# gudgud96/music-fader-nets

Hardware: AMD Instinct MI355X
Metric: event-tokens/sec GM-VAE train, seq256 b256 (higher is better)
Workload: dtype f32/bf16x6; 1 GPU; MusicAttrRegGMVAE train step (fwd+losses+bwd+clip+Adam), hidden 512, z 128, K=2, B=256/GPU, T=256, Tr=64 (BASELINE configs[1]; N>1: DP, RCCL grad all-reduce); global_batch=256, seq_len=256, parallelism=dp1

## Files before the change

### include/fadernets.h

```cpp
#ifndef FADERNETS_H
#define FADERNETS_H

#include <stddef.h>
#include <stdint.h>

#ifdef __cplusplus
extern "C" {
#endif

#define FN_OK 0
#define FN_E_NULL (-1)
#define FN_E_SHAPE (-2)
#define FN_E_ALIGN (-3)
#define FN_E_WORKSPACE (-4)
#define FN_E_COUNT (-5)
#define FN_E_UNSUPPORTED (-6)
#define FN_E_COMM (-7)
#define FN_COMM_ERROR_BASE 2000000

#define FN_MAX_SCANS 8

int fn_version(void);
const char* fn_strerror(int code);

#define FN_GEMM_LEAN 0x10000
#define FN_GEMM_BF16X6 0x20000
#define FN_GEMM_X6_PERWAVE 0x40000
#define FN_GEMM_X6_WIDE 0x80000
#define FN_GEMM_X6_PERTILE 0x100000
size_t fn_gemm_ws_bytes(int M, int N, int splitk);
int fn_gemm_f32(int a_kmajor, int b_kmajor, int M, int N, int K, float alpha,
                const float* A, int lda, const float* B, int ldb, float beta, float* C, int ldc,
                const float* bias, int splitk, float* ws, size_t ws_bytes, void* stream);

typedef struct FnGemmSeg {
    const float* A;
    int32_t lda;
    const float* B;
    int32_t ldb;
    int32_t K;
} FnGemmSeg;
typedef struct FnGemmJob {
    int32_t M, N;
    FnGemmSeg seg[4];
    int32_t n_seg;
    float beta;
    float* C;
    int32_t ldc;
// ... 332 lines not shown
```

### music-fader-nets_amd/_lib.py

```python
import ctypes as C
import os

_HERE = os.path.dirname(os.path.abspath(__file__))
LIB_PATH = os.path.join(_HERE, "libfadernets_hip.so")

FN_MAX_SCANS = 8
ABI_VERSION = 6
GEMM_LEAN = 0x10000
GEMM_BF16X6 = 0x20000
GEMM_X6_WIDE = 0x80000
GEMM_X6_PERTILE = 0x100000
GEMM_X6_PERWAVE = 0x40000
GRU_ROWS_MASK = 0xFF
GRU_ALT_TILING = 0x100
GRU_SYNC_ZEROED = 0x200
GRU_COMPILER_LOOPS = 0x400
GRU_NO_PINGPONG = 0x800
GRU_SPREAD_XCDS = 0x1000
GRU_NO_RS_BWD = 0x2000
GRU_BF16X6 = 0x4000
GRU_X6_SINGLE_GROUP = 0x8000
GRU_X6_BWD_32ROWS = 0x8000
FN_E_NULL, FN_E_SHAPE, FN_E_ALIGN, FN_E_WORKSPACE, FN_E_COUNT = -1, -2, -3, -4, -5
FN_E_UNSUPPORTED = -6
# ... 99 lines not shown


class FnNoteParams(C.Structure):
    _fields_ = [("on_lo", C.c_int32), ("off_lo", C.c_int32), ("n_pitch", C.c_int32), ("shift_lo", C.c_int32), ("n_shift", C.c_int32), ("eos", C.c_int32),
                ("vocab_size", C.c_int32), ("vel_lo", C.c_int32), ("n_vel", C.c_int32), ("default_vel", C.c_int32), ("pad", C.c_int32),
                ("add_eos", C.c_int32), ("reserved", C.c_int32 * 4)]


SIGNATURES = {
    "fn_version": (C.c_int, []),
    "fn_strerror": (C.c_char_p, [C.c_int]),
    "fn_frag3_pack": (C.c_int, [vp, C.c_int, C.c_int, C.c_int, vp, vp]),
    "fn_gemm_ws_bytes": (C.c_size_t, [C.c_int, C.c_int, C.c_int]),
    "fn_gemm_f32": (C.c_int, [C.c_int, C.c_int, C.c_int, C.c_int, C.c_int, C.c_float, vp, C.c_int, vp, C.c_int,
                              C.c_float, vp, C.c_int, vp, C.c_int, vp, C.c_size_t, vp]),
    "fn_gemm_multi": (C.c_int, [C.c_int, C.c_int, C.POINTER(FnGemmJob), C.c_int, vp]),
    "fn_transpose_f32": (C.c_int, [vp, C.c_int, C.c_int, C.c_int, vp, C.c_int, vp]),
    "fn_colsum_ws_bytes": (C.c_size_t, [C.c_int, C.c_int]),
    "fn_colsum_f32": (C.c_int, [vp, C.c_int, C.c_int, C.c_int, C.c_float, vp, vp, C.c_size_t, vp]),
    "fn_colsum_multi": (C.c_int, [C.POINTER(FnColsumJob), C.c_int, vp]),
    "fn_axpy_f32": (C.c_int, [C.c_int64, C.c_float, vp, vp, vp]),
    "fn_sum_f32": (C.c_int, [vp, C.c_int64, C.c_float, vp, vp]),
    "fn_gru_gates_floats": (C.c_size_t, [C.c_int, C.c_int]),
    "fn_frag_floats": (C.c_size_t, [C.c_int, C.c_int]),
    "fn_frag_pack": (C.c_int, [vp, C.c_int, C.c_int, C.c_int, vp, vp]),
    "fn_weight_images": (C.c_int, [C.POINTER(FnWeightImage), C.c_int, vp]),
    "fn_gru_sync_ws_bytes": (C.c_size_t, []),
    "fn_gru_seq_fwd": (C.c_int, [C.POINTER(FnGruFwd), C.c_int, vp]),
    "fn_gru_fwd_x6_ok": (C.c_int, [C.POINTER(FnGruFwd), C.c_int]),
    "fn_gru_cell_f32": (C.c_int, [C.POINTER(FnGruCell), vp]),
# ... 85 lines not shown
```

### music-fader-nets_amd/csrc/gemm.hip

```cpp
#include <type_traits>
#include <utility>

#include "common.h"
#include "mma_core.h"
#include "x6w_core.h"

namespace {

constexpr int NT = 256;
constexpr int PF_DEPTH = 2;

template <int BM, int BN, int BK, int WM, int WN, bool AKC, bool BKC>
__global__ __launch_bounds__(NT) void gemm_kernel(int M, int N, int K, float alpha, const float* __restrict__ A, long lda,
                                                  const float* __restrict__ B, long ldb, float beta, float* __restrict__ C,
                                                  long ldc, const float* __restrict__ bias, int ksplit_len,
                                                  float* __restrict__ slabs) {
    constexpr int TM = BM / WM / 16, TN = BN / WN / 16;
    using SA = Stage<BM, BK, AKC, NT>;
    using SB = Stage<BN, BK, BKC, NT>;
    extern __shared__ __attribute__((aligned(16))) float smem[];

    const int ntn = (N + BN - 1) / BN, ntm = (M + BM - 1) / BM;
    const int tile = fn_xcd_remap(blockIdx.x, ntn * ntm);
    const int tm = tile / ntn, tn = tile % ntn;
// ... 525 lines not shown
        for (int e = 0; e < 4; ++e) x6w_cut_row<RN>(dst, e, fa[decltype(SET)::value]);
    };
    auto fused = [&](auto LS, int lblk, auto CS, int, int stage) __attribute__((always_inline)) {
        const float* p0 = base + 32 * lblk;
        u32x4* dst = lds + stage * X6W_STAGE + ps * X6W_SET + r + 16 * q;
#pragma unroll
        for (int e = 0; e < 4; ++e) {
            ld_row(LS, p0, e);
            x6w_cut_row<RN>(dst, e, fa[decltype(CS)::value]);
            __builtin_amdgcn_sched_barrier(0);
        }
    };
    x6w_trips<NS, 2, false>(nblk, request, cut, fused);
}

__global__ __launch_bounds__(X6W_NT) void gemm_nt_x6w_kernel(int M, int N, int K, float alpha, const float* __restrict__ A, long lda,
                                                              const float* __restrict__ B, long ldb, float beta, float* __restrict__ C, long ldc,
                                                              const float* __restrict__ bias) {
    extern __shared__ __attribute__((aligned(16))) u32x4 x6w_lds[];
    const int ntn = N >> 7, ntiles = ntn * (M >> 7);
    const int lane = threadIdx.x & 63, wave = __builtin_amdgcn_readfirstlane(threadIdx.x >> 6);
    const int nblk = K >> 5;
    if (wave >= 4) {
        const int ps = wave & 3;
#pragma unroll 1
        for (int v = blockIdx.x; v < ntiles; v += gridDim.x) {
            const int tile = fn_xcd_remap(v, ntiles);
            const int mb = (tile / ntn) * 128, nb = (tile % ntn) * 128;
            if (ps < 2) x6w_produce_nt<false>(x6w_lds, A + (long)(mb + 64 * ps) * lda, lda, ps, lane, nblk);
            else x6w_produce_nt<true>(x6w_lds, B + (long)(nb + 64 * (ps - 2)) * ldb, ldb, ps, lane, nblk);
        }
        return;
    }
    const int wm = (wave >> 1) & 1, wn = wave & 1;
    const int li = lane & 15, lg = lane >> 4;
#pragma unroll 1
    for (int v = blockIdx.x; v < ntiles; v += gridDim.x) {
        const int tile = fn_xcd_remap(v, ntiles);
        const int mb = (tile / ntn) * 128, nb = (tile % ntn) * 128;
        f32x4 acc[4][4];
#pragma unroll
        for (int a = 0; a < 4; ++a)
#pragma unroll
            for (int b = 0; b < 4; ++b) acc[a][b] = (f32x4){0.f, 0.f, 0.f, 0.f};
// ... 629 lines not shown
                           B, (long)ldb, beta, C, (long)ldc, bias, klen, slabs);                                           \
    }
    if (ak && bk) FN_GEMM_LAUNCH(true, true)
    else if (ak && !bk) FN_GEMM_LAUNCH(true, false)
    else if (!ak && !bk) FN_GEMM_LAUNCH(false, false)
    else FN_GEMM_LAUNCH(false, true)
#undef FN_GEMM_LAUNCH
    FN_CHECK_LAUNCH();
    if (splitk > 1) {
        launch_slab_reduce(st, slabs, splitk, M, N, alpha, beta, C, (long)ldc, bias);
        FN_CHECK_LAUNCH();
    }
    return FN_OK;
}

}

extern "C" {

int fn_out_head_f32(const float* h, int ldh, const float* W, int ldw, const float* bias, int B, int T, int V, int H, const int32_t* target,
                    float grad_scale, float* nll_rows, float* dlogits, int ld, void* stream) {
    if (!h || !W || !bias || !target) return FN_E_NULL;
    if (B <= 0 || T <= 0 || V <= 0 || H <= 0 || ldh < H || ldw < H) return FN_E_SHAPE;
    if (V > OH_BN) return FN_E_UNSUPPORTED;
    if (dlogits && (ld < V || ld > OH_BN || (ld & 3))) return FN_E_SHAPE;
    if (dlogits && (((uintptr_t)dlogits) & 15)) return FN_E_ALIGN;
    const long R = (long)B * T;
    if (R > 0x7fffffff) return FN_E_SHAPE;
    const size_t lds = out_head_lds_bytes();
    if (const int rc = fn_set_max_lds<out_head_kernel>((int)lds, FN_E_SHAPE)) return rc;
// ... 87 lines not shown
        if (rc != FN_OK) return rc;
    } else {
        hipLaunchKernelGGL(f.lean ? gemm_tn_lean_kernel : gemm_tn_kernel, tn_grid(ntm * ntn, splitk), dim3(NT), 0, st, M, N, K, alpha, A, lda, B, ldb, beta, C,
                           ldc, bias, klen, slabs, A2, lda2, msplit);
    }
    FN_CHECK_LAUNCH();
    if (splitk > 1) {
        launch_slab_reduce(st, slabs, splitk, M, N, alpha, beta, C, ldc, bias);
        FN_CHECK_LAUNCH();
    }
    return FN_OK;
}

size_t fn_gemm_ws_bytes(int M, int N, int splitk) { return splitk > 1 ? (size_t)splitk * M * N * sizeof(float) : 0; }

int fn_gemm_f32(int a_kmajor, int b_kmajor, int M, int N, int K, float alpha, const float* A, int lda, const float* B, int ldb,
                float beta, float* C, int ldc, const float* bias, int splitk, float* ws, size_t ws_bytes, void* stream) {
    if (!A || !B || !C) return FN_E_NULL;
    if (M <= 0 || N <= 0 || K <= 0 || lda <= 0 || ldb <= 0 || ldc < N) return FN_E_SHAPE;
    const SplitkFlags f(splitk);
    const bool lean = f.lean, x6 = f.x6;
    const int x6_mode = f.x6_mode;
    splitk = f.splitk;
    if (splitk > 1 && (!ws || ws_bytes < fn_gemm_ws_bytes(M, N, splitk))) return FN_E_WORKSPACE;
    hipStream_t st = (hipStream_t)stream;
    if (!a_kmajor && !b_kmajor && (lda % 4) == 0 && (ldb % 4) == 0 && lda >= 4 && ldb >= 4 &&
        (((((uintptr_t)A) | ((uintptr_t)B)) & 15) == 0))
        return launch_tn(f, st, M, N, K, alpha, A, (long)lda, B, (long)ldb, beta, C, (long)ldc, bias, ws, (const float*)nullptr, 0L, 0);
    if (x6 && a_kmajor && b_kmajor && splitk <= 1 && (M % 128) == 0 && (N % 128) == 0 && (K % 32) == 0 && K >= 128 && (lda % 4) == 0 && (ldb % 4) == 0 &&
        (ldc % 4) == 0 && (((((uintptr_t)A) | ((uintptr_t)B) | ((uintptr_t)C) | ((uintptr_t)bias)) & 15) == 0) && (long)(M / 128) * (N / 128) >= 128) {
        const size_t lds = (size_t)X6W_STAGES * X6W_STAGE * 16;
        if (const int rc = fn_set_max_lds<gemm_nt_x6w_kernel>((int)lds, FN_E_SHAPE)) return rc;
        const int ntiles = (M / 128) * (N / 128), cus = fn_cu_count();
        const int grid = (ntiles > cus && cus >= 8 && (cus & 7) == 0 && !(x6_mode & FN_GEMM_X6_PERTILE)) ? cus : ntiles;
        hipLaunchKernelGGL(gemm_nt_x6w_kernel, dim3(grid), dim3(X6W_NT), lds, st, M, N, K, alpha, A, (long)lda, B, (long)ldb, beta, C, (long)ldc, bias);
        FN_CHECK_LAUNCH();
        return FN_OK;
    }
    if (a_kmajor && b_kmajor && splitk <= 1 && (M % 128) == 0 && (N % 128) == 0 && (K % 16) == 0 && K >= 64 && (lda % 4) == 0 && (ldb % 4) == 0 &&
        (ldc % 4) == 0 && (((((uintptr_t)A) | ((uintptr_t)B) | ((uintptr_t)C) | ((uintptr_t)bias)) & 15) == 0) &&
        (long)M * lda < (1L << 30) && (long)N * ldb < (1L << 30) && (long)(M / 128) * (N / 128) >= 256) {
        if (lean)
            hipLaunchKernelGGL((gemm_nt_direct_kernel<1, 4>), dim3((M / 128) * (N / 128)), dim3(NT), 0, st, M, N, K, alpha, A, (long)lda, B, (long)ldb, beta, C,
                               (long)ldc, bias);
        else
            hipLaunchKernelGGL((gemm_nt_direct_kernel<4, 2>), dim3((M / 128) * (N / 128)), dim3(NT), 0, st, M, N, K, alpha, A, (long)lda, B, (long)ldb, beta, C,
                               (long)ldc, bias);
        FN_CHECK_LAUNCH();
        return FN_OK;
    }
    if (N <= 16 && a_kmajor && b_kmajor && splitk <= 1 && M >= 64)
        return launch_gemm<64, 16, 16, 4, 1>(a_kmajor, b_kmajor, M, N, K, alpha, A, lda, B, ldb, beta, C, ldc, bias, splitk, ws, st);
// ... 91 lines not shown
```

### music-fader-nets_amd/csrc/gru.hip

```cpp
#include <cstdio>

#include "gru_layout.h"
#include "x6w_core.h"

#ifdef FN_TIMING
__device__ unsigned long long fn_dbg[64 * 8];
#define FN_STAMP(k)                                                                                   \
    do {                                                                                              \
        if (blockIdx.x < 64 && threadIdx.x == 0) fn_dbg[blockIdx.x * 8 + (k)] = __builtin_readcyclecounter(); \
    } while (0)
extern "C" int fn_dbg_read(unsigned long long* host) {
    return (int)hipMemcpyFromSymbol(host, HIP_SYMBOL(fn_dbg), sizeof(unsigned long long) * 64 * 8);
}
#else
#define FN_STAMP(k)
#endif

namespace {

constexpr int NT = 256;

struct FwdStep {
    const float* w_frag;
    const float* b_hh;
// ... 378 lines not shown
        for (int e = 0; e < 2; ++e) {
            const float v = x[2 * j + e];
            hi[e] = fn_rn16(v);
            r1[e] = v - hi[e];
            mi[e] = fn_rn16(r1[e]);
            r2[e] = r1[e] - mi[e];
        }
        h[j] = (__float_as_uint(hi[0]) >> 16) | (__float_as_uint(hi[1]) & 0xffff0000u);
        m[j] = (__float_as_uint(mi[0]) >> 16) | (__float_as_uint(mi[1]) & 0xffff0000u);
        l[j] = (__float_as_uint(r2[0]) >> 16) | (__float_as_uint(r2[1]) & 0xffff0000u);
    }
#pragma unroll
    for (int j = 0; j < 4; ++j) { o[j] = h[j]; o[256 + j] = m[j]; o[512 + j] = l[j]; }
}

__global__ void frag3_pack_kernel(const float* __restrict__ src, int rows, int K, long ld, unsigned* __restrict__ dst) {
    const long total = (long)((rows + 15) & ~15) * (K >> 3);
    for (long i = blockIdx.x * (long)blockDim.x + threadIdx.x; i < total; i += (long)gridDim.x * blockDim.x) frag3_item(src, rows, K, ld, 1, dst, i);
}

constexpr int WI_MAX_JOBS = 56;
struct WiJob {
    const float* src;
    float* dst;
    int R, C, ld, kind;
};
struct WiArgs {
    WiJob job[WI_MAX_JOBS];
};

// ... 9 lines not shown
                const int r = r0 + j, c = c0 + tx;
                t[j][tx] = (r < J.R && c < J.C) ? J.src[(long)r * J.ld + c] : 0.f;
            }
            __syncthreads();
            for (int j = ty; j < 32; j += 8) {
                const int c = c0 + j, r = r0 + tx;
                if (r < J.R && c < J.C) J.dst[(long)c * J.R + r] = t[tx][j];
            }
            __syncthreads();
        }
        return;
    }
    if (J.kind == 5) {
        const long total = (long)J.R * J.C;
        for (long i = blockIdx.x * 256L + threadIdx.x; i < total; i += (long)gridDim.x * 256L) J.dst[i] = J.src[(i / J.C) * J.ld + (i % J.C)];
        return;
    }
    if (J.kind >= 3) {
        const int rows = J.kind == 3 ? J.R : J.C, K = J.kind == 3 ? J.C : J.R;
        const long total = (long)((rows + 15) & ~15) * (K >> 3);
        if (J.kind == 3)
            for (long i = blockIdx.x * 256L + threadIdx.x; i < total; i += (long)gridDim.x * 256L)
                frag3_item<false>(J.src, rows, K, (long)J.ld, 1L, reinterpret_cast<unsigned*>(J.dst), i);
        else
            for (long i = blockIdx.x * 256L + threadIdx.x; i < total; i += (long)gridDim.x * 256L)
                frag3_item<true>(J.src, rows, K, 1L, (long)J.ld, reinterpret_cast<unsigned*>(J.dst), i);
        return;
    }
    const int rows = J.kind == 1 ? J.R : J.C, K = J.kind == 1 ? J.C : J.R;
    const int rows16 = (rows + 15) & ~15, NC = K >> 5;
// ... 943 lines not shown
    auto k = gru_cell_kernel<BM, WM, WN>;
    if (const int rc = fn_set_max_lds<gru_cell_kernel<BM, WM, WN>>((int)lds, FN_E_SHAPE)) return rc;
    const int tiles = ((a.B + BM - 1) / BM) * (a.H / 32);
    hipLaunchKernelGGL(k, dim3(tiles), dim3(NT), lds, st, a);
    FN_CHECK_LAUNCH();
    return FN_OK;
}

extern "C" int fn_weight_images(const FnWeightImage* jobs, int n_jobs, void* stream) {
    if (!jobs) return FN_E_NULL;
    if (n_jobs <= 0 || n_jobs > WI_MAX_JOBS) return FN_E_COUNT;
    WiArgs a;
    for (int j = 0; j < n_jobs; ++j) {
        const FnWeightImage& d = jobs[j];
        if (!d.src || !d.dst) return FN_E_NULL;
        if (d.rows <= 0 || d.cols <= 0 || d.ld < d.cols || d.kind < 0 || d.kind > 5) return FN_E_SHAPE;
        if ((d.kind == 1 || d.kind == 3) && (d.cols % 32)) return FN_E_SHAPE;
        if ((d.kind == 2 || d.kind == 4) && (d.rows % 32)) return FN_E_SHAPE;
        if (d.kind != 0 && (((uintptr_t)d.dst) & 15)) return FN_E_ALIGN;
        a.job[j] = WiJob{d.src, d.dst, d.rows, d.cols, d.ld, d.kind};
    }
    hipLaunchKernelGGL(weight_images_kernel, dim3(128, n_jobs), dim3(256), 0, (hipStream_t)stream, a);
    FN_CHECK_LAUNCH();
    return FN_OK;
}

extern "C" int fn_frag3_pack(const float* src, int rows, int K, int ld, void* dst, void* stream) {
    if (!src || !dst) return FN_E_NULL;
    if (rows <= 0 || K <= 0 || (K % 32) != 0 || ld < K) return FN_E_SHAPE;
    if (((uintptr_t)dst) & 15) return FN_E_ALIGN;
    const long total = (long)((rows + 15) & ~15) * (K >> 3);
    const int blocks = (int)((total + 255) / 256 < 2048 ? (total + 255) / 256 : 2048);
// ... 277 lines not shown
```

### music-fader-nets_amd/decode.py

```python
import numpy as np
import torch

from .constrain import Constraints, constraint_buffers, constraint_stats, load_constraints
from .engine import E_VOCAB, LOGIT_LD


def _is_int(v):
    return isinstance(v, (int, np.integer)) and not isinstance(v, (bool, np.bool_))


def _is_finite(v):
    return isinstance(v, (int, float, np.integer, np.floating)) and not isinstance(v, (bool, np.bool_)) and bool(np.isfinite(v))


def _check_steps(steps, bools=True):
    if not (isinstance(steps, (int, np.integer)) if bools else _is_int(steps)) or steps < 1:
        raise ValueError("steps: a positive int, got %r" % (steps,))


def _force_mask(force, steps):
    _check_steps(steps)
    if _is_int(force):
        if not 0 <= int(force) <= steps:
            raise ValueError("force = P forces the first P steps: 0 <= P <= %d, got %d" % (steps, int(force)))
# ... 63 lines not shown
    return full, P


def _init_state(eng, rows, prefix):
    P, H = eng.p, eng.H
    h0g = eng.buf(prefix + "h0g", (rows.shape[0], H))
    eng.ops.gemm(rows, P["linear_init_global.weight"], h0g, bias=P["linear_init_global.bias"])
    rbg = eng.buf(prefix + "rbg", (rows.shape[0], 3 * H))
    eng.ops.gemm(rows, P["grucell_g.weight_ih"][:, E_VOCAB:], rbg)
    return h0g, rbg


def _arith_key(eng):
    ops = eng.ops
    return (bool(getattr(ops, "dw_x6", False) and getattr(ops, "cell_x6", False)), getattr(ops, "cell_x6_rows", None),
            bool(getattr(ops, "x6_per_tile", False)), bool(getattr(ops, "nt_x6", True)))


def _token_buffers(z, steps, want_logp, forced=None, params=None, con=None):
    return dict(zs=z.clone(), fs=None if forced is None else forced.clone(), ps=None if params is None else params.to(z.device),
                cb=None if con is None else constraint_buffers(con, z.shape[0], z.device),
                tokens=torch.zeros(z.shape[0], steps, dtype=torch.int32, device=z.device),
                logp=torch.empty(z.shape[0], steps, E_VOCAB, device=z.device) if want_logp else None)


def _graph_replay(eng, cache, key, build, body, bounded, inputs, con=None, repeat=1):
    ent = cache.get(key)
    if ent is None:
        bufs = build()
        body(bufs, True)
        g = torch.cuda.CUDAGraph()
# ... 377 lines not shown
```

### music-fader-nets_amd/engine.py

```python
import math

import torch

E_VOCAB, R_DIMS, N_DIMS, C_DIMS = 342, 3, 16, 24
LOGIT_LD = 352


def ops_sort(eng, key, tokens, V):
    n = tokens.numel() + 2 * (V + 1) + 2
    img = eng.buf("sort_img_" + key, (n,), torch.int32) if tokens.is_cuda else None
    return eng.ops.token_sort(tokens, V, img)


class Engine:
    def __init__(self, ops, params, hidden, zdim, n_component, device):
        self.ops = ops
        self.p = params
        self.H, self.Z, self.K = hidden, zdim, n_component
        self.ZG = 2 * zdim + C_DIMS
        self.dev = torch.device(device)
        self._bufs = {}
        self.tab = {}
        self.whh_f = {}
        self.whh_f3 = {}
# ... 191 lines not shown
                    jobs.append(("copy", w[:, V:], self.wz[key]))
        if getattr(self.ops, "dw_x6", False) and H == 512:
            for key, (pfx, sfx, V) in self._gru_sets().items():
                w_hh = self.p[pfx + "weight_hh" + sfx]
                self.whh_f3[key] = self.buf("whhf3_" + key, (self.ops.frag_floats(3 * H, H) * 3 // 2,))
                jobs.append(("frag3", w_hh, self.whh_f3[key]))
                if need_backward:
                    self.whh_t3[key] = self.buf("whht3_" + key, (self.ops.frag_floats(H, 3 * H) * 3 // 2,))
                    jobs.append(("frag3_t", w_hh, self.whh_t3[key]))
        else:
            self.whh_f3.clear()
            self.whh_t3.clear()
        self.ops.weight_images(jobs)
        if need_backward:
            self.ops.transpose(self.p["linear_out_g.weight"], self.wout_t[:, :E_VOCAB])

    def encode(self, d, save=True):
        ops, P, H, Z = self.ops, self.p, self.H, self.Z
        B, T = d.shape
        scans, hall = [], {}
        for e in ("r", "n"):
            for key, sfx, rev in ((e, "_l0", 0), (e + "_reverse", "_l0_reverse", 1)):
                pfx = "gru_%s." % e
                hall[key] = self.buf("enc_h_" + key, (T, B, H))
                scans.append(dict(B=B, T=T, H=H, reverse=rev, w_hh_frag=self.whh_f[key], w_hh_frag3=self.whh_f3.get(key), b_hh=P[pfx + "bias_hh" + sfx],
                                  b_ih=P[pfx + "bias_ih" + sfx], gx_table=self.tab[key], idx=d, idx_shift=0,
                                  h_all=hall[key], gates=self.buf("enc_g_" + key, (T, ops.gates_floats(B, H))) if save else None))
        ops.gru_seq_fwd(scans)
        pre = {"h_all": hall, "gates": {sc_key: sc["gates"] for sc_key, sc in zip(hall, scans)}}
        jobs = []
# ... 127 lines not shown
                        c["h0_frag"] = img
        for k, part in enumerate(launches):
            if k >= 2:
                self.lane_wait("main", "aux%d" % (k & 1))
            if part:
                ops.gru_seq_fwd(part, persistent=pd, **xkw)
            if k < nch:
                t0, t1 = starts[k], min(T, starts[k] + CH)
                lane = "aux%d" % (k & 1)
                self.lane_wait(lane, "main")
                with Engine._Lane(self, True, lane):
                    if k == 0:
                        for src, img in prepack:
                            (ops.frag3_pack if x6 else ops.frag_pack)(src, img)
                    ops.gemm(hx0[t0:t1].view(-1, H), P["grucell_g_2.weight_ih"], gx2[t0:t1].view(-1, 3 * H), bias=P["grucell_g_2.bias_ih"],
                             lean=self.lean_proj, **({} if self.proj_x6 else {"nt_x6": False}))
        logits = self.buf("g_logits", (T * B, LOGIT_LD), zero_init=True)
        if head:
            ops.gemm(hx1.view(T * B, H), P["linear_out_g.weight"], logits[:, :E_VOCAB], bias=P["linear_out_g.bias"])
        return dict(zc=zc, h0g=h0g, rbg=rbg, hx0=hx0, g1=g1, gx2=gx2, hx1=hx1, g2=g2, logits=logits)

    def decoders(self, d, r, n, c, z_r, z_n, save=True, head=True, sd_logits=True):
        if self._fill_ok(d.shape[1], r.shape[1]):
            sd = self.sub_decoders_fwd(r, n, z_r, z_n, save, defer=True)
            dec = self.global_decoder_tf(d, self.pack_zc(z_r, z_n, c), save, head, fill={e: sd[e].pop("scan") for e in ("r", "n")}, more_jobs=sd.pop("init_jobs"))
            if sd_logits:
                self._sub_decoder_logits(sd, r.shape[1], r.shape[0])
        else:
            sd = self.sub_decoders_fwd(r, n, z_r, z_n, save)
            dec = self.global_decoder_tf(d, self.pack_zc(z_r, z_n, c), save, head)
        dec["sd"] = sd
# ... 64 lines not shown
        if h0 is not None:
            ops.gru_dwhh(dgx2[:B], dgn2[:B], h0, dW, beta=1.0)
        db = G[pfx + "bias_hh" + sfx]
        self.colsum(rs[:, : 2 * H], db[: 2 * H])
        self.colsum(rsn, db[2 * H:])

    def _splitk(self, rows):
        return self.splitk_big if rows >= 8192 else (8 if rows >= 4096 else (4 if rows >= 1024 else 1))

    def _bwd_global_decoder_scans(self, S, fill=None, before_first_launch=None):
        ops, P, H = self.ops, self.p, self.H
        dec = S["dec"]
        B, T = S["d"].shape
        dlog = dec["logits"]
        dhx1 = self.buf("g_dhx1", (T, B, H))
        ops.gemm(dlog, self.wout_t, dhx1.view(T * B, H), a_k=True, b_k=True)
        if before_first_launch is not None:
            before_first_launch()
        dgx2 = self.buf("g_dgx2", (T, B, 3 * H))
        dghn2 = self.buf("g_dghn2", (T, B, H))
        dhx0 = self.buf("g_dhx0", (T, B, H))
        dgx1 = self.buf("g_dgx1", (T, B, 3 * H))
        dghn1 = self.buf("g_dghn1", (T, B, H))
        rs2, rsn2 = self.zbuf("g_rs2", (B, 3 * H)), self.zbuf("g_rsn2", (B, H))
        drb_g, rsn_g = self.zbuf("g_drb", (B, 3 * H)), self.zbuf("g_rsn1", (B, H))
        l2 = dict(B=B, T=T, H=H, w_hh_t_frag=self.whh_t["g2"], w_hh_t_frag3=self.whh_t3.get("g2"), h0=dec["hx0"][0], h_all=dec["hx1"], gates=dec["g2"], dh_ext=dhx1,
                  dgx_all=dgx2, dghn_all=dghn2, scratch=self.buf("g_scr2", (B, H)), dgx_rowsum=rs2, dghn_rowsum=rsn2, tag="dec_l2")
        l1 = dict(B=B, T=T, H=H, w_hh_t_frag=self.whh_t["g"], w_hh_t_frag3=self.whh_t3.get("g"), h0=dec["h0g"], h_all=dec["hx0"], gates=dec["g1"], dh_ext=dhx0,
                  dgx_all=dgx1, dghn_all=dghn1, scratch=self.buf("g_scr1", (B, H)), dgx_rowsum=drb_g, dghn_rowsum=rsn_g, tag="dec_l1")
        CH = self.chunk
        carry = {k: [self.buf("carry_%s_%d" % (k, i), (B, H)) for i in range(2)] for k in ("l2", "l1")}
# ... 23 lines not shown
                self.lane_wait("main", "auxb%d" % (k & 1))
                part.append(chunk("l1", l1, js[k - 2]))
            if k >= nch and "r" in fch and k - nch < len(fch["r"]):
                part.append(fch["r"][k - nch])
            if part:
                bkw = {}
                if pd and self.dec_bwd_budget and getattr(ops, "dw_x6", False) and getattr(ops, "bwd_x6", False) and len(part) == 2 \
                        and ops.gru_bwd_x6_ok(part, self.dec_bwd_budget):
                    bkw = {"cu_budget": self.dec_bwd_budget}
                ops.gru_seq_bwd(part, persistent=pd, **bkw)
            if k < nch:
                t0, t1 = js[k], min(T, js[k] + CH)
                lane = "auxb%d" % (k & 1)
                self.lane_wait(lane, "main")
                with Engine._Lane(self, True, lane):
                    ops.gemm(dgx2[t0:t1].view(-1, 3 * H), self.wih2_t, dhx0[t0:t1].view(-1, H), a_k=True, b_k=True)
                    if t0 == 0:
                        ops.axpy(1.0, carry["l2"][0], dhx0[0])
        return dict(dgx1=dgx1, dghn1=dghn1, dgx2=dgx2, dghn2=dghn2, rs2=rs2, rsn2=rsn2, drb_g=drb_g, rsn_g=rsn_g, dh0_g=carry["l1"][0])

    def _bwd_global_decoder_params(self, G, S, gd, flush=True):
        ops, H = self.ops, self.H
        dec = S["dec"]
        B, T = S["d"].shape
        sk_T = self._splitk(T * B)
        dlog = dec["logits"]
        hx1f, hx0f = dec["hx1"].view(T * B, H), dec["hx0"].view(T * B, H)
        dgx1, dghn1, dgx2, dghn2, rs2, rsn2, drb_g, rsn_g, dh0_g = (gd[k] for k in ("dgx1", "dghn1", "dgx2", "dghn2", "rs2", "rsn2", "drb_g", "rsn_g", "dh0_g"))
        ln = self.lean_dw
        ops.gemm(dlog[:, :E_VOCAB], hx1f, G["linear_out_g.weight"], a_k=False, b_k=False, splitk=42 if T * B >= 32768 else sk_T, lean=ln)
        self.colsum(dlog[:, :E_VOCAB], G["linear_out_g.bias"])
# ... 185 lines not shown
```

### music-fader-nets_amd/hipops.py

```python
import ctypes as C

import torch

from . import _lib, arith


def _p(t):
    return None if t is None else C.c_void_p(t.data_ptr())


def _chk(t, dtype=torch.float32, name="tensor"):
    if t is None:
        return
    if not t.is_cuda:
        raise RuntimeError("%s must live on the GPU (got %s): the HIP path has no CPU fallback" % (name, t.device))
    if t.dtype != dtype:
        raise RuntimeError("%s must be %s, got %s" % (name, dtype, t.dtype))


def _mat(t, name):
    _chk(t, name=name)
    if t.dim() != 2 or (t.shape[1] > 1 and t.stride(1) != 1):
        raise RuntimeError("%s must be 2-D with contiguous rows, got shape %s strides %s" % (name, tuple(t.shape), t.stride()))
    ld = t.stride(0) if t.shape[0] > 1 else max(t.shape[1], t.stride(0))
# ... 10 lines not shown
class HipOps:

    name = "hip"

    def __init__(self, device):
        self.lib = _lib.load()
        self.device = torch.device(device)
        if self.device.type != "cuda":
            raise RuntimeError("HipOps needs a GPU device")
        self._ws = {}
        self._retired = []
        self.cell_variant = 0
        self.dw_x6 = arith.default() == arith.BF16X6
        self.x6_wide = True
        self.nt_x6 = True
        self.x6_per_tile = False
        self.cell_x6_rows = 2048
        self.cell_x6 = True
        self.x6_perwave = False
        self.bwd_x6 = True
        self.variant = 0
        self.lane = ""

    def stream(self):
        return C.c_void_p(torch.cuda.current_stream(self.device).cuda_stream)

    def workspace(self, nbytes, tag="ws"):
        tag = self.lane + tag
        cur = self._ws.get(tag)
        if cur is None or cur.numel() * 4 < nbytes:
            if cur is not None:
                self._retired.append(cur)
            cur = torch.empty((max(nbytes, 4) + 3) // 4, dtype=torch.float32, device=self.device)
            self._ws[tag] = cur
        return cur

    def gemm(self, A, B, Cm, a_k=True, b_k=True, alpha=1.0, beta=0.0, bias=None, splitk=1, lean=False, nt_x6=True):
        pa, ar, ac, lda = _mat(A, "A")
        pb, br, bc, ldb = _mat(B, "B")
        pc, M, N, ldc = _mat(Cm, "C")
        K = ac if a_k else ar
        if (ar if a_k else ac) != M or (br if b_k else bc) != N or (bc if b_k else br) != K:
            raise RuntimeError("gemm shape mismatch A%s B%s C%s a_k=%s b_k=%s" % (tuple(A.shape), tuple(B.shape), tuple(Cm.shape), a_k, b_k))
        _chk(bias, name="bias")
        ws, wsb = None, 0
        x6 = _lib.GEMM_BF16X6 if (self.dw_x6 and not a_k and not b_k and K >= 1024) else 0
        if x6:
            splitk, x6 = self._x6_mode(splitk, N, K, x6)
        elif self.dw_x6 and self.nt_x6 and nt_x6 and a_k and b_k and splitk <= 1 and M % 128 == 0 and N % 128 == 0 and K % 32 == 0 and K >= 128 and (M // 128) * (N // 128) >= 128:
            x6 = _lib.GEMM_BF16X6
            if self.x6_per_tile:
                x6 |= _lib.GEMM_X6_PERTILE
        if splitk > 1:
            wsb = self.lib.fn_gemm_ws_bytes(M, N, splitk & 0xffff)
            ws = self.workspace(wsb, "gemm")
        _lib.check(self.lib.fn_gemm_f32(int(a_k), int(b_k), M, N, K, alpha, pa, lda, pb, ldb, beta, pc, ldc, _p(bias),
                                        splitk | (_lib.GEMM_LEAN if lean else 0) | x6,
                                        _p(ws), wsb, self.stream()), "fn_gemm_f32")

    def _x6_mode(self, splitk, N, K, x6):
        if self.x6_wide == "force":
            if not self.x6_perwave:
                x6 |= _lib.GEMM_X6_WIDE
        elif self.x6_wide and N >= 256 and splitk > 1 and K >= 32768:
            splitk *= 2
            if not self.x6_perwave:
                x6 |= _lib.GEMM_X6_WIDE
# ... 66 lines not shown

    def gates_floats(self, B, H):
        return int(self.lib.fn_gru_gates_floats(B, H))

    def frag_floats(self, rows, K):
        return int(self.lib.fn_frag_floats(rows, K))

    def frag_pack(self, src, dst):
        ps, rows, K, ld = _mat(src, "src")
        _dense(dst, name="dst")
        if dst.numel() < self.frag_floats(rows, K):
            raise RuntimeError("frag_pack: dst too small")
        _lib.check(self.lib.fn_frag_pack(ps, rows, K, ld, _p(dst), self.stream()), "fn_frag_pack")

    def weight_images(self, jobs):
        kinds = {"transpose": 0, "frag": 1, "frag_t": 2, "frag3": 3, "frag3_t": 4, "copy": 5}
        for i0 in range(0, len(jobs), 56):
            part = jobs[i0:i0 + 56]
            arr = (_lib.FnWeightImage * len(part))()
            for d, (kind, src, dst) in zip(arr, part):
                ps, R, Cc, ld = _mat(src, "src")
                _dense(dst, name="dst")
                need = {"transpose": lambda: R * Cc, "copy": lambda: R * Cc, "frag": lambda: self.frag_floats(R, Cc), "frag_t": lambda: self.frag_floats(Cc, R),
                        "frag3": lambda: self.frag_floats(R, Cc) * 3 // 2, "frag3_t": lambda: self.frag_floats(Cc, R) * 3 // 2}[kind]()
                if dst.numel() < need:
                    raise RuntimeError("weight_images: dst too small for %s of %s" % (kind, tuple(src.shape)))
                d.src, d.dst, d.rows, d.cols, d.ld, d.kind = ps, _p(dst), R, Cc, ld, kinds[kind]
            _lib.check(self.lib.fn_weight_images(arr, len(part), self.stream()), "fn_weight_images")

    def _frag_ws(self, tag, i, n):
        return self.workspace(4 * n, "%s%d" % (tag, i))[:n]

    SYNC_REGIONS = 64

    def begin_capture(self):
        for ent in self.__dict__.get("_sync_pools", {}).values():
            ent["next"] = 0

    def _sync_region(self):
# ... 606 lines not shown
```

### music-fader-nets_amd/trainer.py

```python
import contextlib
import math
import os

import numpy as np

import torch

from .engine import E_VOCAB

DECODER_PREFIXES = ("linear_out_g.", "grucell_g_2.", "grucell_g.", "linear_init_global.", "gru_d_r.", "gru_d_n.",
                    "linear_out_r.", "linear_out_n.", "linear_init_r.", "linear_init_n.")

S_CE_X, S_CE_R, S_CE_N, S_L_R, S_L_N, S_TERMS_R, S_TERMS_N, S_LEN = 0, 1, 2, 3, 4, 5, 9, 16


def beta_schedule(step, beta):
    return 0.0 if step < 1000 else min((step - 10000) / 10000 * beta, beta)


class FlatParams:

    def __init__(self, model):
        named = model.used_parameters()
        dec = [kp for kp in named if kp[0].startswith(DECODER_PREFIXES)]
# ... 245 lines not shown

    def step_device(self, step, batch, eps):
        m = self.model
        self._sync_step_counter(step)
        beta0 = beta_schedule(step, self.beta)
        B = batch[0].shape[0]
        Bg = B if self.dist is None else self.dist.global_batch(B)
        self._dev_step = step + 1
        self.flat.t += 1
        if not self.use_graph:
            m.engine()
            self._gather_densities(batch, None)
            self._step_body(step, batch, eps)
            m._weights_version = (m._version, m._param_versions())
            return beta0, Bg
        key = (tuple(batch[0].shape), tuple(batch[1].shape), batch[6] is not None, bool(getattr(m.engine().ops, "dw_x6", False)))
        st = self._static.get(key)
        if st is None:
            st = dict(batch=[None if t is None else t.clone() for t in batch], eps=[None if e is None else e.clone() for e in eps], runs=0)
            self._static[key] = st
        groups = {}
        for dst, src in zip(st["batch"] + st["eps"], list(batch) + list(eps)):
            if dst is not None and dst.data_ptr() != src.data_ptr():
                if src.device == dst.device and src.dtype == dst.dtype and src.shape == dst.shape:
                    g = groups.setdefault(dst.dtype, ([], []))
                    g[0].append(dst), g[1].append(src)
                else:
                    dst.copy_(src, non_blocking=True)
        for dsts, srcs in groups.values():
            if len(dsts) > 1:
                torch._foreach_copy_(dsts, srcs, non_blocking=True)
# ... 74 lines not shown
```

Measured before the change: 3.887 million event-tokens/s.

## Presplit bf16x6 weight images for NT x6 GEMMs once per weight refresh

Adds a weight-image kind that pre-splits the B-side weights into the bf16x3 hi/mid/lo LDS layout. A new NT x6 GEMM entry point has its B producer waves copy that image straight into LDS instead of loading fp32 and splitting each time. It is wired into the GRU layer-2 input projection and the two backward GEMMs that use the output and input-hidden transposes. This removes repeated split work and fp32 B loads per tile, at the cost of extra weight-image memory and a packing pass after every optimizer step.

Result: no change. 3.914 million event-tokens/s, median of 6 (+0.7%).

```diff
diff --git a/include/fadernets.h b/include/fadernets.h
--- a/include/fadernets.h
+++ b/include/fadernets.h
@@ -32,6 +32,8 @@
 int fn_gemm_f32(int a_kmajor, int b_kmajor, int M, int N, int K, float alpha,
                 const float* A, int lda, const float* B, int ldb, float beta, float* C, int ldc,
                 const float* bias, int splitk, float* ws, size_t ws_bytes, void* stream);
+int fn_gemm_nt_x6p_f32(int M, int N, int K, float alpha, const float* A, int lda, const void* B_image, float beta, float* C, int ldc,
+                       const float* bias, int flags, void* stream);
 
 typedef struct FnGemmSeg {
     const float* A;
diff --git a/music-fader-nets_amd/_lib.py b/music-fader-nets_amd/_lib.py
--- a/music-fader-nets_amd/_lib.py
+++ b/music-fader-nets_amd/_lib.py
@@ -137,6 +137,7 @@
     "fn_gemm_ws_bytes": (C.c_size_t, [C.c_int, C.c_int, C.c_int]),
     "fn_gemm_f32": (C.c_int, [C.c_int, C.c_int, C.c_int, C.c_int, C.c_int, C.c_float, vp, C.c_int, vp, C.c_int,
                               C.c_float, vp, C.c_int, vp, C.c_int, vp, C.c_size_t, vp]),
+    "fn_gemm_nt_x6p_f32": (C.c_int, [C.c_int, C.c_int, C.c_int, C.c_float, vp, C.c_int, vp, C.c_float, vp, C.c_int, vp, C.c_int, vp]),
     "fn_gemm_multi": (C.c_int, [C.c_int, C.c_int, C.POINTER(FnGemmJob), C.c_int, vp]),
     "fn_transpose_f32": (C.c_int, [vp, C.c_int, C.c_int, C.c_int, vp, C.c_int, vp]),
     "fn_colsum_ws_bytes": (C.c_size_t, [C.c_int, C.c_int]),
diff --git a/music-fader-nets_amd/csrc/gemm.hip b/music-fader-nets_amd/csrc/gemm.hip
--- a/music-fader-nets_amd/csrc/gemm.hip
+++ b/music-fader-nets_amd/csrc/gemm.hip
@@ -563,6 +563,36 @@
     x6w_trips<NS, 2, false>(nblk, request, cut, fused);
 }
 
+FN_DEVINL void x6w_produce_nt_img(u32x4* __restrict__ lds, const u32x4* __restrict__ img, int ps, int lane, int nblk) {
+    constexpr int NS = X6W_NS, NV = X6W_SET / 64;
+    u32x4 fa[NS][NV];
+    const u32x4* base = img + lane;
+    auto request = [&](auto SET, int blk) __attribute__((always_inline)) {
+        const u32x4* p0 = base + (long)blk * X6W_SET;
+#pragma unroll
+        for (int i = 0; i < NV; ++i) fa[decltype(SET)::value][i] = p0[i * 64];
+    };
+    auto cut = [&](auto SET, int, int stage) __attribute__((always_inline)) {
+        u32x4* dst = lds + stage * X6W_STAGE + ps * X6W_SET + lane;
+#pragma unroll
+        for (int i = 0; i < NV; ++i) dst[i * 64] = fa[decltype(SET)::value][i];
+    };
+    auto fused = [&](auto LS, int lblk, auto CS, int, int stage) __attribute__((always_inline)) {
+        const u32x4* p0 = base + (long)lblk * X6W_SET;
+        u32x4* dst = lds + stage * X6W_STAGE + ps * X6W_SET + lane;
+#pragma unroll
+        for (int e = 0; e < 4; ++e) {
+#pragma unroll
+            for (int i = 3 * e; i < 3 * e + 3; ++i) fa[decltype(LS)::value][i] = p0[i * 64];
+#pragma unroll
+            for (int i = 3 * e; i < 3 * e + 3; ++i) dst[i * 64] = fa[decltype(CS)::value][i];
+            __builtin_amdgcn_sched_barrier(0);
+        }
+    };
+    x6w_trips<NS, 2, false>(nblk, request, cut, fused);
+}
+
+template <bool BIMG>
 __global__ __launch_bounds__(X6W_NT) void gemm_nt_x6w_kernel(int M, int N, int K, float alpha, const float* __restrict__ A, long lda,
                                                               const float* __restrict__ B, long ldb, float beta, float* __restrict__ C, long ldc,
                                                               const float* __restrict__ bias) {
@@ -577,6 +607,8 @@
             const int tile = fn_xcd_remap(v, ntiles);
             const int mb = (tile / ntn) * 128, nb = (tile % ntn) * 128;
             if (ps < 2) x6w_produce_nt<false>(x6w_lds, A + (long)(mb + 64 * ps) * lda, lda, ps, lane, nblk);
+            else if constexpr (BIMG)
+                x6w_produce_nt_img(x6w_lds, reinterpret_cast<const u32x4*>(B) + (long)((nb >> 6) + (ps - 2)) * nblk * X6W_SET, ps, lane, nblk);
             else x6w_produce_nt<true>(x6w_lds, B + (long)(nb + 64 * (ps - 2)) * ldb, ldb, ps, lane, nblk);
         }
         return;
@@ -1236,6 +1268,18 @@
     return FN_OK;
 }
 
+template <bool BIMG>
+static int launch_nt_x6(int x6_mode, hipStream_t st, int M, int N, int K, float alpha, const float* A, long lda, const float* B, long ldb, float beta,
+                        float* C, long ldc, const float* bias) {
+    const size_t lds = (size_t)X6W_STAGES * X6W_STAGE * 16;
+    if (const int rc = fn_set_max_lds<gemm_nt_x6w_kernel<BIMG>>((int)lds, FN_E_SHAPE)) return rc;
+    const int ntiles = (M / 128) * (N / 128), cus = fn_cu_count();
+    const int grid = (ntiles > cus && cus >= 8 && (cus & 7) == 0 && !(x6_mode & FN_GEMM_X6_PERTILE)) ? cus : ntiles;
+    hipLaunchKernelGGL(gemm_nt_x6w_kernel<BIMG>, dim3(grid), dim3(X6W_NT), lds, st, M, N, K, alpha, A, lda, B, ldb, beta, C, ldc, bias);
+    FN_CHECK_LAUNCH();
+    return FN_OK;
+}
+
 }
 
 extern "C" {
@@ -1353,6 +1397,16 @@
 
 size_t fn_gemm_ws_bytes(int M, int N, int splitk) { return splitk > 1 ? (size_t)splitk * M * N * sizeof(float) : 0; }
 
+int fn_gemm_nt_x6p_f32(int M, int N, int K, float alpha, const float* A, int lda, const void* B_image, float beta, float* C, int ldc, const float* bias,
+                       int flags, void* stream) {
+    if (!A || !B_image || !C) return FN_E_NULL;
+    if (M <= 0 || N <= 0 || K < 128 || lda < K || ldc < N || (M % 128) || (N % 128) || (K % 32) || (lda % 4) || (ldc % 4) ||
+        (long)(M / 128) * (N / 128) < 128 || (flags & ~FN_GEMM_X6_PERTILE) ||
+        (((((uintptr_t)A) | ((uintptr_t)B_image) | ((uintptr_t)C) | ((uintptr_t)bias)) & 15) != 0))
+        return FN_E_SHAPE;
+    return launch_nt_x6<true>(flags, (hipStream_t)stream, M, N, K, alpha, A, (long)lda, static_cast<const float*>(B_image), 0L, beta, C, (long)ldc, bias);
+}
+
 int fn_gemm_f32(int a_kmajor, int b_kmajor, int M, int N, int K, float alpha, const float* A, int lda, const float* B, int ldb,
                 float beta, float* C, int ldc, const float* bias, int splitk, float* ws, size_t ws_bytes, void* stream) {
     if (!A || !B || !C) return FN_E_NULL;
@@ -1368,13 +1422,7 @@
         return launch_tn(f, st, M, N, K, alpha, A, (long)lda, B, (long)ldb, beta, C, (long)ldc, bias, ws, (const float*)nullptr, 0L, 0);
     if (x6 && a_kmajor && b_kmajor && splitk <= 1 && (M % 128) == 0 && (N % 128) == 0 && (K % 32) == 0 && K >= 128 && (lda % 4) == 0 && (ldb % 4) == 0 &&
         (ldc % 4) == 0 && (((((uintptr_t)A) | ((uintptr_t)B) | ((uintptr_t)C) | ((uintptr_t)bias)) & 15) == 0) && (long)(M / 128) * (N / 128) >= 128) {
-        const size_t lds = (size_t)X6W_STAGES * X6W_STAGE * 16;
-        if (const int rc = fn_set_max_lds<gemm_nt_x6w_kernel>((int)lds, FN_E_SHAPE)) return rc;
-        const int ntiles = (M / 128) * (N / 128), cus = fn_cu_count();
-        const int grid = (ntiles > cus && cus >= 8 && (cus & 7) == 0 && !(x6_mode & FN_GEMM_X6_PERTILE)) ? cus : ntiles;
-        hipLaunchKernelGGL(gemm_nt_x6w_kernel, dim3(grid), dim3(X6W_NT), lds, st, M, N, K, alpha, A, (long)lda, B, (long)ldb, beta, C, (long)ldc, bias);
-        FN_CHECK_LAUNCH();
-        return FN_OK;
+        return launch_nt_x6<false>(x6_mode, st, M, N, K, alpha, A, (long)lda, B, (long)ldb, beta, C, (long)ldc, bias);
     }
     if (a_kmajor && b_kmajor && splitk <= 1 && (M % 128) == 0 && (N % 128) == 0 && (K % 16) == 0 && K >= 64 && (lda % 4) == 0 && (ldb % 4) == 0 &&
         (ldc % 4) == 0 && (((((uintptr_t)A) | ((uintptr_t)B) | ((uintptr_t)C) | ((uintptr_t)bias)) & 15) == 0) &&
diff --git a/music-fader-nets_amd/csrc/gru.hip b/music-fader-nets_amd/csrc/gru.hip
--- a/music-fader-nets_amd/csrc/gru.hip
+++ b/music-fader-nets_amd/csrc/gru.hip
@@ -416,6 +416,19 @@
     for (int j = 0; j < 4; ++j) { o[j] = h[j]; o[256 + j] = m[j]; o[512 + j] = l[j]; }
 }
 
+FN_DEVINL void nt6_item(const float* __restrict__ src, int K, long ld, u32x4* __restrict__ dst, long i) {
+    const int nb = K >> 5;
+    const long set = i >> 8;
+    const int e = (int)(i >> 6) & 3, l = (int)i & 63, r = l & 15, q = l >> 4;
+    const float* p = src + ((set / nb) * 64 + 4 * r + e) * ld + (set % nb) * 32 + 8 * q;
+    float x[8];
+#pragma unroll
+    for (int j = 0; j < 8; ++j) x[j] = p[j];
+    u32x4 h, m, lo;
+    fn_split<true>(x, h, m, lo);
+    x6w_put(dst + set * X6W_SET + l, e, h, m, lo);
+}
+
 __global__ void frag3_pack_kernel(const float* __restrict__ src, int rows, int K, long ld, unsigned* __restrict__ dst) {
     const long total = (long)((rows + 15) & ~15) * (K >> 3);
     for (long i = blockIdx.x * (long)blockDim.x + threadIdx.x; i < total; i += (long)gridDim.x * blockDim.x) frag3_item(src, rows, K, ld, 1, dst, i);
@@ -455,6 +468,11 @@
     if (J.kind == 5) {
         const long total = (long)J.R * J.C;
         for (long i = blockIdx.x * 256L + threadIdx.x; i < total; i += (long)gridDim.x * 256L) J.dst[i] = J.src[(i / J.C) * J.ld + (i % J.C)];
+        return;
+    }
+    if (J.kind == 6) {
+        const long total = (long)J.R * (J.C >> 3);
+        for (long i = blockIdx.x * 256L + threadIdx.x; i < total; i += (long)gridDim.x * 256L) nt6_item(J.src, J.C, (long)J.ld, reinterpret_cast<u32x4*>(J.dst), i);
         return;
     }
     if (J.kind >= 3) {
@@ -1428,8 +1446,9 @@
     for (int j = 0; j < n_jobs; ++j) {
         const FnWeightImage& d = jobs[j];
         if (!d.src || !d.dst) return FN_E_NULL;
-        if (d.rows <= 0 || d.cols <= 0 || d.ld < d.cols || d.kind < 0 || d.kind > 5) return FN_E_SHAPE;
-        if ((d.kind == 1 || d.kind == 3) && (d.cols % 32)) return FN_E_SHAPE;
+        if (d.rows <= 0 || d.cols <= 0 || d.ld < d.cols || d.kind < 0 || d.kind > 6) return FN_E_SHAPE;
+        if ((d.kind == 1 || d.kind == 3 || d.kind == 6) && (d.cols % 32)) return FN_E_SHAPE;
+        if (d.kind == 6 && (d.rows % 64)) return FN_E_SHAPE;
         if ((d.kind == 2 || d.kind == 4) && (d.rows % 32)) return FN_E_SHAPE;
         if (d.kind != 0 && (((uintptr_t)d.dst) & 15)) return FN_E_ALIGN;
         a.job[j] = WiJob{d.src, d.dst, d.rows, d.cols, d.ld, d.kind};
diff --git a/music-fader-nets_amd/decode.py b/music-fader-nets_amd/decode.py
--- a/music-fader-nets_amd/decode.py
+++ b/music-fader-nets_amd/decode.py
@@ -101,7 +101,7 @@
 def _arith_key(eng):
     ops = eng.ops
     return (bool(getattr(ops, "dw_x6", False) and getattr(ops, "cell_x6", False)), getattr(ops, "cell_x6_rows", None),
-            bool(getattr(ops, "x6_per_tile", False)), bool(getattr(ops, "nt_x6", True)))
+            bool(getattr(ops, "x6_per_tile", False)), bool(getattr(ops, "nt_x6", True)), bool(getattr(ops, "nt_presplit", False)))
 
 
 def _token_buffers(z, steps, want_logp, forced=None, params=None, con=None):
diff --git a/music-fader-nets_amd/engine.py b/music-fader-nets_amd/engine.py
--- a/music-fader-nets_amd/engine.py
+++ b/music-fader-nets_amd/engine.py
@@ -229,6 +229,18 @@
         self.ops.weight_images(jobs)
         if need_backward:
             self.ops.transpose(self.p["linear_out_g.weight"], self.wout_t[:, :E_VOCAB])
+        self.nt_img = {}
+        if getattr(self.ops, "dw_x6", False) and getattr(self.ops, "nt_presplit", False) and H % 128 == 0 and "grucell_g_2.weight_ih" in self.p:
+            srcs = {"ih2": self.p["grucell_g_2.weight_ih"]}
+            if need_backward:
+                srcs.update(ih2_t=self.wih2_t, out_t=self.wout_t)
+            for key, w in srcs.items():
+                self.nt_img[key] = self.buf("nt6_" + key, (w.shape[0] * w.shape[1] * 3 // 2,))
+            self.ops.weight_images([("nt6", w, self.nt_img[key]) for key, w in srcs.items()])
+
+    def _nt_image(self, key):
+        img = getattr(self, "nt_img", {}).get(key)
+        return {} if img is None else {"b_image": img}
 
     def encode(self, d, save=True):
         ops, P, H, Z = self.ops, self.p, self.H, self.Z
@@ -386,7 +398,7 @@
                         for src, img in prepack:
                             (ops.frag3_pack if x6 else ops.frag_pack)(src, img)
                     ops.gemm(hx0[t0:t1].view(-1, H), P["grucell_g_2.weight_ih"], gx2[t0:t1].view(-1, 3 * H), bias=P["grucell_g_2.bias_ih"],
-                             lean=self.lean_proj, **({} if self.proj_x6 else {"nt_x6": False}))
+                             lean=self.lean_proj, **({} if self.proj_x6 else {"nt_x6": False}), **self._nt_image("ih2"))
         logits = self.buf("g_logits", (T * B, LOGIT_LD), zero_init=True)
         if head:
             ops.gemm(hx1.view(T * B, H), P["linear_out_g.weight"], logits[:, :E_VOCAB], bias=P["linear_out_g.bias"])
@@ -481,7 +493,7 @@
         B, T = S["d"].shape
         dlog = dec["logits"]
         dhx1 = self.buf("g_dhx1", (T, B, H))
-        ops.gemm(dlog, self.wout_t, dhx1.view(T * B, H), a_k=True, b_k=True)
+        ops.gemm(dlog, self.wout_t, dhx1.view(T * B, H), a_k=True, b_k=True, **self._nt_image("out_t"))
         if before_first_launch is not None:
             before_first_launch()
         dgx2 = self.buf("g_dgx2", (T, B, 3 * H))
@@ -535,7 +547,7 @@
                 lane = "auxb%d" % (k & 1)
                 self.lane_wait(lane, "main")
                 with Engine._Lane(self, True, lane):
-                    ops.gemm(dgx2[t0:t1].view(-1, 3 * H), self.wih2_t, dhx0[t0:t1].view(-1, H), a_k=True, b_k=True)
+                    ops.gemm(dgx2[t0:t1].view(-1, 3 * H), self.wih2_t, dhx0[t0:t1].view(-1, H), a_k=True, b_k=True, **self._nt_image("ih2_t"))
                     if t0 == 0:
                         ops.axpy(1.0, carry["l2"][0], dhx0[0])
         return dict(dgx1=dgx1, dghn1=dghn1, dgx2=dgx2, dghn2=dghn2, rs2=rs2, rsn2=rsn2, drb_g=drb_g, rsn_g=rsn_g, dh0_g=carry["l1"][0])
diff --git a/music-fader-nets_amd/hipops.py b/music-fader-nets_amd/hipops.py
--- a/music-fader-nets_amd/hipops.py
+++ b/music-fader-nets_amd/hipops.py
@@ -48,6 +48,7 @@
         self.dw_x6 = arith.default() == arith.BF16X6
         self.x6_wide = True
         self.nt_x6 = True
+        self.nt_presplit = True
         self.x6_per_tile = False
         self.cell_x6_rows = 2048
         self.cell_x6 = True
@@ -69,7 +70,7 @@
             self._ws[tag] = cur
         return cur
 
-    def gemm(self, A, B, Cm, a_k=True, b_k=True, alpha=1.0, beta=0.0, bias=None, splitk=1, lean=False, nt_x6=True):
+    def gemm(self, A, B, Cm, a_k=True, b_k=True, alpha=1.0, beta=0.0, bias=None, splitk=1, lean=False, nt_x6=True, b_image=None):
         pa, ar, ac, lda = _mat(A, "A")
         pb, br, bc, ldb = _mat(B, "B")
         pc, M, N, ldc = _mat(Cm, "C")
@@ -85,6 +86,13 @@
             x6 = _lib.GEMM_BF16X6
             if self.x6_per_tile:
                 x6 |= _lib.GEMM_X6_PERTILE
+            if b_image is not None and self.nt_presplit:
+                _dense(b_image, name="b_image")
+                if b_image.numel() * 2 < 3 * N * K:
+                    raise RuntimeError("gemm: b_image too small for B%s" % (tuple(B.shape),))
+                _lib.check(self.lib.fn_gemm_nt_x6p_f32(M, N, K, alpha, pa, lda, _p(b_image), beta, pc, ldc, _p(bias), x6 & _lib.GEMM_X6_PERTILE,
+                                                       self.stream()), "fn_gemm_nt_x6p_f32")
+                return
         if splitk > 1:
             wsb = self.lib.fn_gemm_ws_bytes(M, N, splitk & 0xffff)
             ws = self.workspace(wsb, "gemm")
@@ -181,7 +189,7 @@
         _lib.check(self.lib.fn_frag_pack(ps, rows, K, ld, _p(dst), self.stream()), "fn_frag_pack")
 
     def weight_images(self, jobs):
-        kinds = {"transpose": 0, "frag": 1, "frag_t": 2, "frag3": 3, "frag3_t": 4, "copy": 5}
+        kinds = {"transpose": 0, "frag": 1, "frag_t": 2, "frag3": 3, "frag3_t": 4, "copy": 5, "nt6": 6}
         for i0 in range(0, len(jobs), 56):
             part = jobs[i0:i0 + 56]
             arr = (_lib.FnWeightImage * len(part))()
@@ -189,7 +197,7 @@
                 ps, R, Cc, ld = _mat(src, "src")
                 _dense(dst, name="dst")
                 need = {"transpose": lambda: R * Cc, "copy": lambda: R * Cc, "frag": lambda: self.frag_floats(R, Cc), "frag_t": lambda: self.frag_floats(Cc, R),
-                        "frag3": lambda: self.frag_floats(R, Cc) * 3 // 2, "frag3_t": lambda: self.frag_floats(Cc, R) * 3 // 2}[kind]()
+                        "frag3": lambda: self.frag_floats(R, Cc) * 3 // 2, "frag3_t": lambda: self.frag_floats(Cc, R) * 3 // 2, "nt6": lambda: R * Cc * 3 // 2}[kind]()
                 if dst.numel() < need:
                     raise RuntimeError("weight_images: dst too small for %s of %s" % (kind, tuple(src.shape)))
                 d.src, d.dst, d.rows, d.cols, d.ld, d.kind = ps, _p(dst), R, Cc, ld, kinds[kind]
diff --git a/music-fader-nets_amd/trainer.py b/music-fader-nets_amd/trainer.py
--- a/music-fader-nets_amd/trainer.py
+++ b/music-fader-nets_amd/trainer.py
@@ -283,7 +283,8 @@
             self._step_body(step, batch, eps)
             m._weights_version = (m._version, m._param_versions())
             return beta0, Bg
-        key = (tuple(batch[0].shape), tuple(batch[1].shape), batch[6] is not None, bool(getattr(m.engine().ops, "dw_x6", False)))
+        key = (tuple(batch[0].shape), tuple(batch[1].shape), batch[6] is not None, bool(getattr(m.engine().ops, "dw_x6", False)),
+               bool(getattr(m.engine().ops, "nt_presplit", False)))
         st = self._static.get(key)
         if st is None:
             st = dict(batch=[None if t is None else t.clone() for t in batch], eps=[None if e is None else e.clone() for e in eps], runs=0)
```
